# LeonOrou/OPF-Graph-Neural-Solver

Measured on AMD Instinct MI355X. Metric: grids/sec (fwd+bwd) on batched case118, K=4, higher is better.
Workload: dtype f32

## Files before the change

opf-graph-neural-solver_amd/csrc/gns_api.hip:

```cpp
#include <atomic>
#include <cmath>
#include <cstring>
#include <cstdlib>
#include <mutex>
#include <vector>
#include "gns_kernels.h"
#include "gns_gridwg.h"

namespace {
struct GnsTuning {
  int fwd_mapping;
  int gw_pack;
  int fwd_waves;
  int fwd_plane;
  int dw_mfma;
  int train_mapping;
  int bwd_variant;
  int team;
  int bwds_mode;
  int bwds_chunks;
  int bwds_save;
};

bool waves_ok(int& w) { return w > 0 && (w & (w - 1)) == 0 && w * 64 <= GNS_FWD_MAX_THREADS; }
bool chunks_ok(int& c) { return c == 0 || gns_part_index(c) >= 0; }
bool as_flag(int& v) { v = v ? 1 : 0; return true; }
int env_int(const char* e) { return std::atoi(e); }
int env_mapping(const char* e) { return !std::strcmp(e, "lane") ? 1 : (!std::strcmp(e, "lds") ? 2 : 0); }
int env_plane(const char* e) { return e[0] == '0' ? 0 : (e[0] == '1' ? 1 : 2); }
int env_flag(const char* e) { return e[0] == '0' ? 0 : 1; }
struct GnsOption {
  const char* name; int GnsTuning::*member; int lo, hi; bool (*check)(int&); const char* env; int (*parse)(const char*);
  bool accepts(int& v) const { return check ? check(v) : (v >= lo && v <= hi); }
};
const GnsOption g_options[] = {
  {"fwd_mapping",   &GnsTuning::fwd_mapping,   0, 2,            nullptr,   "GNS_FWD_MAPPING",   env_mapping},
  {"train_mapping", &GnsTuning::train_mapping, 0, 2,            nullptr,   "GNS_TRAIN_MAPPING", env_mapping},
  {"bwd_variant",   &GnsTuning::bwd_variant,   1, 4,            nullptr,   "GNS_BWD_VARIANT",   env_int},
  {"gw_pack",       &GnsTuning::gw_pack,       0, 16,           nullptr,   "GNS_GW_PACK",       env_int},
  {"fwd_waves",     &GnsTuning::fwd_waves,     0, 0,            waves_ok,  "GNS_FWD_WAVES",     env_int},
  {"fwd_plane",     &GnsTuning::fwd_plane,     0, 2,            nullptr,   "GNS_FWD_PLANE",     env_plane},
  {"dw_mfma",       &GnsTuning::dw_mfma,       0, 0,            as_flag,   "GNS_DW_MFMA",       env_flag},
  {"team",          &GnsTuning::team,          0, GNS_MAX_TEAM, nullptr,   "GNS_TEAM",          env_int},
  {"bwds_mode",     &GnsTuning::bwds_mode,     0, 2,            nullptr,   "GNS_BWDS_MODE",     env_int},
  {"bwds_chunks",   &GnsTuning::bwds_chunks,   0, 0,            chunks_ok, "GNS_BWDS_CHUNKS",   env_int},
  {"bwds_save",     &GnsTuning::bwds_save,     0, 1,            nullptr,   "GNS_BWDS_SAVE",     env_int},
};
GnsTuning make_tuning() {
  GnsTuning t{0, 0, GNS_FWD_THREADS / 64, 2, 1, 0, 4, 0, 1, 0, 1};
  for (const GnsOption& o : g_options)
    if (const char* e = std::getenv(o.env)) { int v = o.parse(e); if (o.accepts(v)) t.*o.member = v; }
  return t;
}
GnsTuning& tuning() {
  static GnsTuning t = make_tuning();
  return t;
}

struct GnsLast {
  int fwd_kernel, fwd_waves, fwd_plane, team, gw_pack;
  int bwd_kernel, dw_mfma, bwds_mode, bwds_chunks, bwds_R, bwd_gw_pack;
  int bwds_save;
};
GnsLast g_last{-1, -1, -1, -1, -1, -1, -1, -1, -1, -1, -1, -1};
struct GnsLastName { const char* name; int GnsLast::*member; };
const GnsLastName g_last_names[] = {
  {"fwd_kernel", &GnsLast::fwd_kernel}, {"fwd_waves", &GnsLast::fwd_waves}, {"fwd_plane", &GnsLast::fwd_plane}, {"team", &GnsLast::team},
  {"gw_pack", &GnsLast::gw_pack}, {"bwd_kernel", &GnsLast::bwd_kernel}, {"dw_mfma", &GnsLast::dw_mfma}, {"bwds_mode", &GnsLast::bwds_mode},
  {"bwds_chunks", &GnsLast::bwds_chunks}, {"bwds_R", &GnsLast::bwds_R}, {"bwd_gw_pack", &GnsLast::bwd_gw_pack},
  {"bwds_save", &GnsLast::bwds_save},
};
void record_forward(int kernel, int waves, int plane, int team, int pack) {
  g_last.fwd_kernel = kernel; g_last.fwd_waves = waves; g_last.fwd_plane = plane; g_last.team = team; g_last.gw_pack = pack;
}
void record_backward(int kernel, int dw_mfma, int mode, int chunks, int R, int pack, int save = 0) {
  g_last.bwd_kernel = kernel; g_last.dw_mfma = dw_mfma; g_last.bwds_mode = mode; g_last.bwds_chunks = chunks; g_last.bwds_R = R;
  g_last.bwd_gw_pack = pack; g_last.bwds_save = save;
}

constexpr int GNS_MAX_DEVICES = 64;
struct GnsDevice {
  int ncu;
  int gw_ready;
  int split_ready;
  int fwd_ready;
};
const GnsDevice& device() {
  static GnsDevice devs[GNS_MAX_DEVICES];
  static std::atomic<int> done[GNS_MAX_DEVICES];
  static std::mutex mu;
  static const GnsDevice none{0, 0, 0, 0};
  int dev = 0;
  if (hipGetDevice(&dev) != hipSuccess) { (void)hipGetLastError(); return none; }
  if (dev < 0 || dev >= GNS_MAX_DEVICES) return none;
  if (!done[dev].load(std::memory_order_acquire)) {
    std::lock_guard<std::mutex> lock(mu);
    if (!done[dev].load(std::memory_order_relaxed)) {
      GnsDevice d{0, 0, 0, 0};
      int n = 0;
      if (hipDeviceGetAttribute(&n, hipDeviceAttributeMultiprocessorCount, dev) == hipSuccess) d.ncu = n;
// ... 276 lines not shown
                   const void* packed_inputs, int64_t Bt, const float* grad_total, const float* grad_last, const float* grad_v,
                   const float* grad_theta, float* grad_params, hipStream_t st, const IgradOut* ig = nullptr) {
  const int N = cfg->n_bus, E = cfg->n_line, K = cfg->K, d = cfg->latent_dim, h = cfg->hidden_dim;
  int rc;
  GnsBwdsArgs A;
  std::memset(&A, 0, sizeof(A));
  A.topo = topo_dev; A.group_topo = group_topo; A.slot_grid = slot_grid;
  A.pt = (const float*)(fw + L.off_pt); A.pn = (const float*)(fw + L.off_pn);
  A.in = packed_inputs ? (const float*)packed_inputs : (const float*)(fw + L.off_in);
  A.state = (const float*)(fw + L.off_state); A.lam = (const float*)(fw + L.off_lam); A.msg = (const float*)(fw + L.off_msg);
  A.g_total = grad_total; A.g_last = grad_last; A.g_v = grad_v; A.g_theta = grad_theta;
  A.adj = (float*)(bw + S.off_adj); A.slots = (float*)(bw + S.off_slots); A.slab = (float*)(bw + S.off_slab);
  fill_backward_families(A, fam);
  A.Bt = Bt; A.G = S.groups; A.slab_floats = S.slab_floats; A.N = N; A.E = E; A.K = K;
  A.C = S.C; A.part_idx = gns_part_index(S.C); A.R = S.R;
  A.RB = (int)(1 + S.mq); A.RBA = (int)S.adj_rows;
  A.mode = cfg->multiple_phi ? tuning().bwds_mode : 2;
  const size_t lds = gns_bwds_phys_lds(N, &A.use_plane);
  if (ig) {
    A.igrad = ig->buf;
    if (hipMemsetAsync(A.igrad, 0, ig->bytes, st) != hipSuccess) return GNS_ELAUNCH;
  }
  A.save_a1 = saves_first_layer(cfg, ig ? GNS_SAVE_IGRAD : 1, group_topo != nullptr) ? 1 : 0;
  record_backward(4, 1, A.mode, A.C, A.R, -1, A.save_a1);
  prof_mark(1, true, st);
  for (int k = K - 1; k >= 0; --k) {
    A.k = k;
    A.gwk = loss_weight(cfg, k);
    rc = gns_launch_bwds_phys(A, lds, st);
    if (rc != GNS_OK) return rc;
    if (ig) {
      rc = gns_launch_bwds_igrad_phys(A, st);
      if (rc != GNS_OK) return rc;
    }
    rc = gns_launch_bwds_sweep(d, h, cfg->multiple_phi, A, st);
    if (rc != GNS_OK) return rc;
  }
  if (ig && (ig->buses || ig->lines || ig->gens)) {
    rc = gns_launch_bwds_igrad_unpack(A, ig->in_buses, ig->in_lines, ig->in_gens, cfg->n_gen, ig->buses, ig->lines, ig->gens, st);
    if (rc != GNS_OK) return rc;
  }
  prof_mark(1, false, st);
  if (!grad_params) return GNS_OK;
  return gns_launch_reduce(A.slab, (float*)(bw + S.off_part), (float*)(bw + S.off_tmp), params, grad_params, S.nslab, S.slab_floats,
                           fam, K, d, h, st);
}
}
// ... 434 lines not shown
```

opf-graph-neural-solver_amd/csrc/gns_backward_split.hip:

```cpp
#include "gns_device.h"
#include "gns_kernels.h"
#include "gns_dw.h"
#include "gns_phys_device.h"

typedef int gns_i8v __attribute__((ext_vector_type(8)));
#ifndef GNS_BWDS_ONE_LAYOUT
#define GNS_BWDS_ONE_LAYOUT 0
#endif
#ifndef GNS_BWDS_WPE
#define GNS_BWDS_WPE 2
#endif
#ifndef GNS_BWDS_KEEP_SLOPES
#define GNS_BWDS_KEEP_SLOPES 1
#endif
#if GNS_BWDS_KEEP_SLOPES
#define GNS_SLOPES(sl) sl
#define GNS_SLOPE_OF(sl, layer, act, u) sl[layer][u]
#else
#define GNS_SLOPES(sl) nullptr
#define GNS_SLOPE_OF(sl, layer, act, u) dlrelu2(act[u])
#endif
#ifndef GNS_BWDS_FRESH_INPUTS
#define GNS_BWDS_FRESH_INPUTS 1
#endif
#ifndef GNS_BWDS_LINE_AHEAD
#define GNS_BWDS_LINE_AHEAD 1
#endif
#ifndef GNS_BWDS_BUS_AHEAD
#define GNS_BWDS_BUS_AHEAD 1
#endif
#ifndef GNS_BWDS_AH_M
#define GNS_BWDS_AH_M 5
#endif
#ifndef GNS_BWDS_AH_M0
#define GNS_BWDS_AH_M0 5
#endif
#ifndef GNS_BWDS_AH_T0
#define GNS_BWDS_AH_T0 4
#endif
#ifndef GNS_BWDS_LASTK_FOLD
#define GNS_BWDS_LASTK_FOLD 0
#endif
#define GNS_BWDS_PHYS_THREADS (GNS_BWDS_PHYS_WAVES * 64)

__global__ void __launch_bounds__(GNS_BWDS_PHYS_THREADS) gns_bwds_phys_kernel(GnsBwdsArgs A) {
  extern __shared__ __attribute__((aligned(16))) float lds[];
  constexpr int W = GNS_BWDS_PHYS_WAVES;
  const int lane = threadIdx.x & 63;
  const int wave = __builtin_amdgcn_readfirstlane(threadIdx.x >> 6);
  const int N = A.N, E = A.E, K = A.K, k = A.k;
  cip topo = (cip)A.topo;
  const long long g = blockIdx.x;
  long long b = g * GNS_LANES + lane;
  bool live = b < A.Bt;
  if (A.group_topo) {
    const int s = A.slot_grid[g * GNS_LANES + lane];
    b = s;
    live = s >= 0 && s < A.Bt;
    if (!gns_group_topo(A.topo, A.group_topo, g, N, E, topo)) return;
  }
  constexpr int pidx = 4;
// ... 206 lines not shown
  static constexpr bool FOLD4 = WIDE && l < 2 && XT + H + 1 <= 16;
  static constexpr bool FOLDM = GwSubWide::NA >= 16 && WIDE && l == 2 && XT + H + 1 <= 16 && H + (OUT - 16) <= 16;

  static constexpr int NT4 = FOLD4 ? 1 : (FOLDM ? 1 : NA4);
  f32x4 T1[NB1], T2, T4[NT4];
  cfp nb, ptl;

  __device__ __forceinline__ void init(const GnsBwdsArgs& A) {
    const long long koff = A.k;
    nb = (cfp)A.pn + A.n_off[C::NPHI + l] + koff * A.n_sz[C::NPHI + l];
    ptl = (cfp)A.pt + A.t_off[C::NPHI + l] + koff * A.t_sz[C::NPHI + l];
    scalar_cache_warm(ptl, A.t_sz[C::NPHI + l]);
#if !GNS_BWDS_ONE_LAYOUT
    scalar_cache_warm(nb, A.n_sz[C::NPHI + l]);
#endif
    const f32x4 z4 = {0.f, 0.f, 0.f, 0.f};
#pragma unroll
    for (int t = 0; t < NB1; ++t) T1[t] = z4;
#pragma unroll
    for (int t = 0; t < NT4; ++t) T4[t] = z4;
    T2 = z4;
  }

  template <bool ACC_GS, bool STEP0, bool IG = false, bool SV = false>
  __device__ __forceinline__ void bus(const GnsBwdsArgs& A, float* rec, int lane, long long g, int n, float g3s, f2 (&xs)[XL],
                                      f2 (&macc)[D / 2], f4& xsum, f2 (&gS)[H / 2], float* park = nullptr) {
    static_assert(!SV || (MULTI && !GNS_BWDS_ONE_LAYOUT && WIDE && 2 * SOFF >= 16 && (FOLD4 || FOLDM)), "saved activations: the (20, 10) windows");
    f2 (&S)[H / 2] = reinterpret_cast<f2 (&)[H / 2]>(xs[SOFF]);
    f2 a1[H / 2], a2[H / 2], g2[H / 2], g1[H / 2];
    if constexpr (SV) load_pairs<H>(A.msg, ((((long long)A.k * A.G + g) * A.N + n) * C::NPHI + fphi) * C::HQ, lane, a1);
    else load_pairs<H>(A.msg, ((((long long)A.k * A.G + g) * A.N + n) * C::NPHI + fphi) * C::HQ, lane, S);
    WFirst wf;
    f2 sl[2][H / 2];
    using TL [[maybe_unused]] = TLay<LIN, H, OUTP>;
#if GNS_BWDS_ONE_LAYOUT
    (void)wf;
    mlp2_fwd<LIN, H>(ptl, xs, a1, a2, NoBG{}, NoLink{}, GNS_SLOPES(sl));
#else
    using LKm = std::conditional_t<STEP0, NoLink, L2>; using LKs = std::conditional_t<STEP0, std::conditional_t<FOLD4, L0, NoLink>, std::conditional_t<FOLD4, L1, L2>>;
    if constexpr (SV) {
      mlp2_fwd_l2<LIN, H>(ptl, a1, a2, std::conditional_t<STEP0, NoLink, L0>{nullptr, nb, &wf}, GNS_SLOPES(sl));
    } else if constexpr (STEP0) {
      f2 u4[H / 2];
      const f2 (&st)[2] = reinterpret_cast<const f2 (&)[2]>(xs[0]);
      const f2 (&tl)[(LIN - 4 - D + 1) / 2] = reinterpret_cast<const f2 (&)[(LIN - 4 - D + 1) / 2]>(xs[SOFF]);
      phi_head<4, H>(ptl, st, u4);
      phi_tail<LIN, H, 4 + D>(ptl, u4, tl, a1, a2, NoBG{}, NoLink{}, GNS_SLOPES(sl));
    } else {
      mlp2_fwd<LIN, H>(ptl, xs, a1, a2, NoBG{}, L0{nullptr, nb, &wf}, GNS_SLOPES(sl));
    }
#endif
#if GNS_BWDS_ONE_LAYOUT
    if constexpr (l == 2) {
// ... 107 lines not shown

  __device__ __forceinline__ void flush(const GnsBwdsArgs& A, int lane, float* slab) {
    const long long koff = A.k;
    constexpr int ob1 = LIN * H, oW2 = ob1 + H, ob2 = oW2 + H * H, oW4 = ob2 + H, ob4 = oW4 + OUT * H;
    float* lb_ = slab + A.g_off[C::NPHI + l] + koff * A.g_sz[C::NPHI + l];
    static_for<0, NB1>([&](auto t_) { constexpr int t = decltype(t_)::value;
      gws_flush(lane, T1[t], lb_, [&](int c, int il) {
        const bool lastw = WIDE && t == NB1 - 1;
        const int i = 16 * t + il;
        if (c < H) return (lastw && il >= XT) ? -1 : (i < LIN ? c * LIN + i : (i == LIN ? ob1 + c : -1));
        if (FOLD4 && lastw && c == H && il >= XT && il <= XT + H) return il - XT < H ? oW4 + (il - XT) : ob4;
        if (FOLDM && lastw && c >= H && c < H + (OUT - 16) && il >= XT && il <= XT + H) { const int j = 16 + c - H; return il - XT < H ? oW4 + j * H + (il - XT) : ob4 + j; }
        return -1; }, true); });
    gws_flush(lane, T2, lb_, [&](int c, int il) { return c < H ? (il < H ? oW2 + c * H + il : (il == H ? ob2 + c : -1)) : -1; }, true);
    if constexpr (FOLDM)
      gws_flush(lane, T4[0], lb_, [&](int c, int il) { return il < H ? oW4 + c * H + il : (il == H ? ob4 + c : -1); }, true);
    else if constexpr (!FOLD4)
    static_for<0, NA4>([&](auto t_) { constexpr int t = decltype(t_)::value;
      gws_flush(lane, T4[t], lb_, [&](int c, int il) { const int j = 12 * t + c; return (c < 12 && j < OUT) ? (il < H ? oW4 + j * H + il : (il == H ? ob4 + j : -1)) : -1; }, true); });
  }
};

struct BwdsLineRows { f4 a, b; };
__device__ __forceinline__ BwdsLineRows bwds_line_rows(const float* IN, long long row_ein, int p, int lane) {
  return BwdsLineRows{*row_ptr(IN, row_ein + 3LL * p, lane), *row_ptr(IN, row_ein + 3LL * p + 1, lane)};
}

template <int D, int H, bool MULTI, int PF>
struct BwdsPhi : BwdsShape<D, H, MULTI> {
  using B = BwdsShape<D, H, MULTI>;
  using C = typename B::C;
  using SW = typename B::SW;
  using L0 = typename B::L0; using L2 = typename B::L2;
  static constexpr int XL = B::XL, PIN = B::PIN, NDM = B::NDM, NDMF = B::NDMF;
  static constexpr bool WIDE = B::WIDE;

  f32x4 TP1, TP2, TPm[NDMF];
  cfp pnb, ptb;

  __device__ __forceinline__ void init(const GnsBwdsArgs& A) {
    const long long koff = A.k;
    pnb = (cfp)A.pn + A.n_off[PF] + koff * A.n_sz[PF];
    ptb = (cfp)A.pt + A.t_off[PF] + koff * A.t_sz[PF];
    scalar_cache_warm(ptb, A.t_sz[PF]);
#if !GNS_BWDS_ONE_LAYOUT
    scalar_cache_warm(pnb, A.n_sz[PF]);
#endif
    const f32x4 z4 = {0.f, 0.f, 0.f, 0.f};
#pragma unroll
    for (int t = 0; t < NDMF; ++t) TPm[t] = z4;
    TP1 = z4; TP2 = z4;
  }

  template <bool STEP0, bool IG = false, bool LA = false, bool SV = false>
  __device__ __forceinline__ void bus(const GnsBwdsArgs& A, float* rec, int lane, const f2 (&xs)[XL], const f2 (&gS)[H / 2],
                                      f2 (&macc)[D / 2], int p0, int p1, long long row_ein, const BwdsLineRows& first) {
    if (p0 >= p1) return;
    const float* IN = A.in;
    const f2 (&m)[D / 2] = reinterpret_cast<const f2 (&)[D / 2]>(xs[2]);
    WFirst wf;
    (void)wf;
    f2 uh[H / 2], G1[H / 2];
    if constexpr (WIDE)
      static_for<0, (D - 16) / 2>([&](auto j_) { constexpr int j = decltype(j_)::value; gws_putB<SW>(rec, lane, 8 + (PIN - D + 2) / 2 + j, m[8 + j]); });
    if constexpr (STEP0) {
#pragma unroll
      for (int j = 0; j < H / 2; ++j) uh[j] = f2{0.f, 0.f};
    } else {
      phi_head<D, H>(ptb, m, uh);
    }
#pragma unroll
    for (int j = 0; j < H / 2; ++j) G1[j] = f2{0.f, 0.f};
    f4 ca, cb;
    if constexpr (LA) { ca = first.a; cb = first.b; }
    for (int p = p0; p < p1; ++p) {
      f4 na, nb, ea, eb;
      if constexpr (LA) {
        na = *row_ptr(IN, row_ein + 3LL * min(p + 1, p1 - 1), lane); nb = *row_ptr(IN, row_ein + 3LL * min(p + 1, p1 - 1) + 1, lane);
        ea = ca; eb = cb;
      } else {
        ea = *row_ptr(IN, row_ein + 3LL * p, lane); eb = *row_ptr(IN, row_ein + 3LL * p + 1, lane);
      }
      const f2 xt[3] = {f2{ea.x, ea.y}, f2{ea.z, ea.w}, f2{eb.x, 0.f}};
      f2 a1[H / 2], a2[H / 2], g2[H / 2], g1[H / 2];
      f2 sl[2][H / 2];
#if GNS_BWDS_ONE_LAYOUT
      phi_tail<PIN, H, D>(ptb, uh, xt, a1, a2, NoBG{}, NoLink{}, GNS_SLOPES(sl));
#pragma unroll
      for (int u = 0; u < H / 2; ++u) g2[u] = gS[u] * GNS_SLOPE_OF(sl, 1, a2, u);
      bwd_rows_fwd_layout<H, H>(ptb + TLay2<PIN, H>::oW2, g2, g1);
#else
      phi_tail<PIN, H, D>(ptb, uh, xt, a1, a2, NoBG{}, L0{nullptr, pnb, &wf}, GNS_SLOPES(sl));
      if constexpr (SV) {
        f2* const S = const_cast<f2*>(&xs[B::SOFF]);
#pragma unroll
        for (int u = 0; u < H / 2; ++u) S[u] += a2[u];
      }
#pragma unroll
      for (int u = 0; u < H / 2; ++u) g2[u] = gS[u] * GNS_SLOPE_OF(sl, 1, a2, u);
      bwd_rows<H, H>(pnb, g2, g1, NoBG{}, L2{&wf, nullptr, nullptr});
#endif
// ... 53 lines not shown
    gws_flush(lane, TP2, pb_, [&](int c, int il) { return c < H ? (il < H ? pW2 + c * H + il : (il == H ? pb2 + c : -1)) : -1; }, true);
    static_for<0, NDMF>([&](auto t_) { constexpr int t = decltype(t_)::value;
      gws_flush(lane, TPm[t], pb_, [&](int c, int il) { const int i = 16 * t + il; return (c < H && i < D) ? c * PIN + i : -1; }, true); });
  }
};

template <int D, int H, bool MULTI, int FAMS, bool GROUPED, bool IG>
struct BwdsMeasured { static constexpr bool value = MULTI && D == 20 && H == 10 && (FAMS == 3 || FAMS == 4) && !GROUPED && !IG; };
template <int D>
struct BwdsTop { f4 a0, s0; f2 m[D / 2], q0[D / 2], q2[D / 2]; };
template <int D, int H, bool MULTI, int FAMS, bool STEP0, bool GROUPED, bool IG>
struct BwdsAhead {
#if GNS_BWDS_BUS_AHEAD
  static constexpr int value = !BwdsMeasured<D, H, MULTI, FAMS, GROUPED, IG>::value ? 0 : (FAMS == 4 ? (STEP0 ? GNS_BWDS_AH_M0 : GNS_BWDS_AH_M) : (STEP0 ? GNS_BWDS_AH_T0 : 0));
#else
  static constexpr int value = 0;
#endif
};

template <bool SV, int H> struct BwdsPark { static __device__ __forceinline__ float* get() { return nullptr; } };
template <int H> struct BwdsPark<true, H> {
  static __device__ __forceinline__ float* get() { __shared__ __attribute__((aligned(16))) float park[2 * H * GNS_LANES]; return park; }
};
template <int D, int H, bool MULTI, int FAMS, bool STEP0, bool GROUPED, bool IG, bool SV = false>
__global__ void __launch_bounds__(64) __attribute__((amdgpu_waves_per_eu(GNS_BWDS_WPE))) gns_bwds_sweep_kernel(GnsBwdsArgs A) {
  static_assert(!SV || BwdsMeasured<D, H, MULTI, FAMS, GROUPED, IG>::value, "saved activations: the measured shape only");
  using C = GnsDims<D, H, MULTI>;
  static_assert(MULTI || FAMS == 7, "the single phi is reversed after all three L nets");
  constexpr int RB = C::RB, MQ = C::MQ, RBA = 4 + 6 * MQ;
  constexpr bool HAS_T = FAMS & 1, HAS_V = FAMS & 2, HAS_M = FAMS & 4;
  constexpr int SLOT = HAS_M ? 2 : (HAS_T ? 0 : 1);
  constexpr int LIN = C::LF_IN, XL = (LIN + 1) / 2;
  constexpr int RECF = 64 * (D > 16 ? GwSubWide::RS : GwSub::RS);
  __shared__ __attribute__((aligned(16))) float rec[RECF];
  float* const park = BwdsPark<SV, H>::get();
  const int lane = threadIdx.x;
  const long long GB = (A.G + A.R - 1) / A.R;
  const long long bid = blockIdx.x;
  const long long gb = bid % GB;
  const int c = (int)(bid / GB);
  const int N = A.N, E = A.E, K = A.K, k = A.k;
  cip topo = (cip)A.topo;
  cip part = topo + topo[TH_PART] + A.part_idx * (GNS_MAXP + 1), in_ptr = topo + topo[TH_IN_PTR], is_gen = topo + topo[TH_IS_GEN];
  int n0 = part[c], n1 = part[c + 1];
  const long long g0 = gb * A.R, g1 = (g0 + A.R < A.G) ? g0 + A.R : A.G;
  float* slab = A.slab + (gb * A.C + c) * A.slab_floats;
  const bool lastk = k == K - 1;
  constexpr bool LA = BwdsMeasured<D, H, MULTI, FAMS, GROUPED, IG>::value && (GNS_BWDS_LINE_AHEAD == 1 || (GNS_BWDS_LINE_AHEAD == 2 && FAMS == 4));
  constexpr bool ZERO_M = HAS_M || (GNS_BWDS_LASTK_FOLD && MULTI && HAS_T && !GROUPED && !IG);
  if (ZERO_M && lastk) {
    float* z0 = slab + A.g_off[C::NPHI + 2] + (long long)(K - 1) * A.g_sz[C::NPHI + 2];
    for (int i = lane; i < (int)A.g_sz[C::NPHI + 2]; i += 64) z0[i] = 0.f;
    if constexpr (MULTI) {
      float* z1 = slab + A.g_off[2] + (long long)(K - 1) * A.g_sz[2];
      for (int i = lane; i < (int)A.g_sz[2]; i += 64) z1[i] = 0.f;
    }
    if (!HAS_T && !HAS_V) return;
  }
// ... 2 lines not shown
  BwdsL<D, H, MULTI, 1> lv;
  BwdsPhi<D, H, MULTI, MULTI ? 2 : 0> pm;
  BwdsPhi<D, H, MULTI, MULTI ? 1 : 0> pt;
  BwdsPhi<D, H, MULTI, 0> pv;
  if constexpr (HAS_M) { lm.init(A); pm.init(A); }
  if constexpr (HAS_T) { lt.init(A); if constexpr (MULTI) pt.init(A); }
  if constexpr (HAS_V) { lv.init(A); if constexpr (MULTI) pv.init(A); }
  constexpr bool step0 = STEP0;
  const int par = k & 1, parn = par ^ 1;
  const bool m2_live = (A.mode == 2) || k + 1 < K - 1;
  const long long R = gns_in_rows(N, E);

  for (long long g = g0; g < g1; ++g) {
    if constexpr (GROUPED) {
      if (!gns_group_topo(A.topo, A.group_topo, g, N, E, topo)) continue;
      part = topo + topo[TH_PART] + A.part_idx * (GNS_MAXP + 1); in_ptr = topo + topo[TH_IN_PTR]; is_gen = topo + topo[TH_IS_GEN];
      n0 = part[c]; n1 = part[c + 1];
    }
    const long long row_ein = g * R + 3LL * N;
    auto state_row = [&](int slot, int n) { return (((long long)slot * A.G + g) * N + n) * RB; };
    constexpr int AH = BwdsAhead<D, H, MULTI, FAMS, STEP0, GROUPED, IG>::value;
    auto request = [&](int nn, BwdsTop<D>& t) {
      const long long arn = (g * N + nn) * RBA, mrn = arn + 4 + (long long)parn * 3 * MQ;
      if constexpr (AH & 4) { t.a0 = *row_ptr(A.adj, arn, lane); t.s0 = *row_ptr(A.state, state_row(k, nn), lane); }
      if constexpr (AH & 2) load_pairs<D>(A.state, state_row(k, nn) + 1, lane, t.m);
      if constexpr (AH & 1) { load_pairs<D>(A.adj, mrn, lane, t.q0); load_pairs<D>(A.adj, mrn + (m2_live ? 2 : 0) * MQ, lane, t.q2); }
    };
    BwdsTop<D> nx;
    if constexpr (AH != 0) { if (n0 < n1) request(n0, nx); }
    for (int n = n0; n < n1; ++n) {
      const long long ar = (g * N + n) * RBA, rr = state_row(k, n);
      const f4 a0 = [&]() { if constexpr (AH & 4) return nx.a0; else return *row_ptr(A.adj, ar, lane); }();
      const f4 s0 = [&]() { if constexpr (AH & 4) return nx.s0; else return *row_ptr(A.state, rr, lane); }();
      f2 xs[XL];
      f2 (&m)[D / 2] = reinterpret_cast<f2 (&)[D / 2]>(xs[2]);
      if constexpr (AH & 2) {
#pragma unroll
        for (int i = 0; i < D / 2; ++i) m[i] = nx.m[i];
      } else {
        load_pairs<D>(A.state, (step0 ? state_row(0, n0) : rr) + 1, lane, m);
      }
      f2 macc[D / 2];
      if (HAS_M && !lastk) {
        const long long mr = ar + 4 + (long long)parn * 3 * MQ;
        if (A.mode == 2) {
          load_pairs<D>(A.adj, mr + 2 * MQ, lane, macc);
        } else {
          f2 p0v[D / 2];
          if constexpr (AH & 1) {
#pragma unroll
            for (int i = 0; i < D / 2; ++i) { p0v[i] = nx.q0[i]; macc[i] = nx.q2[i]; }
          } else {
            load_pairs<D>(A.adj, mr, lane, p0v);
            load_pairs<D>(A.adj, mr + (m2_live ? 2 : 0) * MQ, lane, macc);
          }
          if (A.mode == 0) {
            f2 p1v[D / 2];
            load_pairs<D>(A.adj, mr + MQ, lane, p1v);
#pragma unroll
            for (int i = 0; i < D / 2; ++i) macc[i] = m2_live ? (macc[i] + p0v[i]) + p1v[i] : p0v[i] + p1v[i];
          } else {
#pragma unroll
            for (int i = 0; i < D / 2; ++i) macc[i] = m2_live ? macc[i] + p0v[i] : p0v[i];
          }
        }
      } else {
#pragma unroll
        for (int i = 0; i < D / 2; ++i) macc[i] = f2{0.f, 0.f};
      }
      auto ahead = [&]() { if constexpr (AH != 0) request(min(n + 1, n1 - 1), nx); };
      f4 xsum = f4{0.f, 0.f, 0.f, 0.f};
      const int p0 = in_ptr[n], p1 = in_ptr[n + 1];
      xs[0] = f2{s0.x, s0.y}; xs[1] = f2{s0.z, s0.w};
      xs[XL - 1] = f2{(float)(p1 - p0), 1.f};
      f2 gS[H / 2];
      const float g3v = is_gen[n] ? 0.f : a0.x;
      auto fresh = [&]() {
#if GNS_BWDS_FRESH_INPUTS
        pin_all(xs);
#endif
      };
      BwdsLineRows lr;
      auto first = [&]() { if constexpr (LA) lr = bwds_line_rows(A.in, row_ein, max(min(p0, E - 1), 0), lane); };
      constexpr int SOFF = 2 + D / 2;
      auto zs = [&]() {
        if constexpr (SV) {
#pragma unroll
          for (int j = 0; j < H / 2; ++j) xs[SOFF + j] = f2{0.f, 0.f};
        }
      };
      if constexpr (MULTI) {
        if constexpr (HAS_M) { if (!lastk) { first(); zs(); fresh(); lm.template bus<false, STEP0, IG, SV>(A, rec, lane, g, n, 0.f, xs, macc, xsum, gS, park); ahead(); fresh(); pm.template bus<STEP0, IG, LA, SV>(A, rec, lane, xs, gS, macc, p0, p1, row_ein, lr); if constexpr (SV) lm.finish(rec, park, lane, xs); } }
        if constexpr (HAS_T) { first(); zs(); fresh(); lt.template bus<false, STEP0, IG, SV>(A, rec, lane, g, n, a0.y, xs, macc, xsum, gS, park); if constexpr (!HAS_M) ahead(); fresh(); pt.template bus<STEP0, IG, LA, SV>(A, rec, lane, xs, gS, macc, p0, p1, row_ein, lr); if constexpr (SV) lt.finish(rec, park, lane, xs); }
        if constexpr (HAS_V) { if (!is_gen[n]) { first(); zs(); fresh(); lv.template bus<false, STEP0, IG, SV>(A, rec, lane, g, n, g3v, xs, macc, xsum, gS, park); fresh(); pv.template bus<STEP0, IG, LA, SV>(A, rec, lane, xs, gS, macc, p0, p1, row_ein, lr); if constexpr (SV) lv.finish(rec, park, lane, xs); } }
      } else {
#pragma unroll
        for (int j = 0; j < H / 2; ++j) gS[j] = f2{0.f, 0.f};
        if (!lastk) { fresh(); lm.template bus<true, STEP0, IG>(A, rec, lane, g, n, 0.f, xs, macc, xsum, gS); }
        first(); fresh(); lt.template bus<true, STEP0, IG>(A, rec, lane, g, n, a0.y, xs, macc, xsum, gS);
        if (!is_gen[n]) { fresh(); lv.template bus<true, STEP0, IG>(A, rec, lane, g, n, g3v, xs, macc, xsum, gS); }
        fresh(); pm.template bus<STEP0, IG, LA>(A, rec, lane, xs, gS, macc, p0, p1, row_ein, lr);
      }
      if constexpr (!step0) {
        *row_ptr(A.adj, ar + 1 + SLOT, lane) = xsum;
        store_pairs<D>(A.adj, ar + 4 + (par * 3 + SLOT) * MQ, lane, macc);
      } else if constexpr (IG) {
        *row_ptr(A.adj, ar + 1 + SLOT, lane) = xsum;
      }
    }
  }
  if constexpr (HAS_M) { if (!lastk) lm.flush(A, lane, slab); if (MULTI ? !lastk : true) pm.flush(A, lane, slab); }
  if constexpr (HAS_T) { lt.flush(A, lane, slab); if constexpr (MULTI) pt.flush(A, lane, slab); }
  if constexpr (HAS_V) { lv.flush(A, lane, slab); if constexpr (MULTI) pv.flush(A, lane, slab); }
}

__global__ void __launch_bounds__(GNS_BWDS_PHYS_THREADS) gns_bwds_igrad_phys_kernel(GnsBwdsArgs A) {
  __shared__ float red[GNS_BWDS_PHYS_WAVES * GNS_LANES];
  constexpr int W = GNS_BWDS_PHYS_WAVES;
  const int lane = threadIdx.x & 63;
  const int wave = __builtin_amdgcn_readfirstlane(threadIdx.x >> 6);
  const int N = A.N, E = A.E, k = A.k;
  cip topo = (cip)A.topo;
  const long long g = blockIdx.x;
  constexpr int pidx = 4;
  const cip in_ptr = topo + topo[TH_IN_PTR], out_ptr = topo + topo[TH_OUT_PTR], q2p = topo + topo[TH_Q2P], is_gen = topo + topo[TH_IS_GEN],
// ... 185 lines not shown

size_t gns_bwds_phys_lds(int N, int* use_plane) {
  const size_t red = (size_t)GNS_BWDS_PHYS_WAVES * GNS_LANES * 4;
  const size_t plane = (size_t)N * GNS_LANES * 4;
  const int level = red + 3 * plane <= (size_t)160 * 1024 ? 2 : (red + 2 * plane <= (size_t)160 * 1024 ? 1 : 0);
  if (use_plane) *use_plane = level;
  return red + (level == 2 ? 3 : (level == 1 ? 2 : 0)) * plane;
}

int gns_launch_bwds_phys(const GnsBwdsArgs& A, size_t lds, hipStream_t st) {
  hipLaunchKernelGGL(gns_bwds_phys_kernel, dim3((unsigned)A.G), dim3(GNS_BWDS_PHYS_THREADS), lds, st, A);
  return hipGetLastError() == hipSuccess ? GNS_OK : GNS_ELAUNCH;
}

int gns_launch_bwds_sweep(int d, int h, int multi, const GnsBwdsArgs& A, hipStream_t st) {
  const long long GB = (A.G + A.R - 1) / A.R;
  const unsigned blocks = (unsigned)(GB * A.C);
  const bool fold_m = GNS_BWDS_LASTK_FOLD && A.k == A.K - 1 && !A.group_topo && !A.igrad;
#define GNS_SWEEP1(DD, HH, MM, FAMS, GR, IG) do { if (A.k == 0) hipLaunchKernelGGL((gns_bwds_sweep_kernel<DD, HH, MM, FAMS, true, GR, IG>), dim3(blocks), dim3(64), 0, st, A); \
                                                 else hipLaunchKernelGGL((gns_bwds_sweep_kernel<DD, HH, MM, FAMS, false, GR, IG>), dim3(blocks), dim3(64), 0, st, A); } while (0)
#define GNS_SWEEP(DD, HH, MM, FAMS) do { if (A.group_topo) GNS_SWEEP1(DD, HH, MM, FAMS, true, false); \
                                         else if (A.igrad) GNS_SWEEP1(DD, HH, MM, FAMS, false, true); \
                                         else GNS_SWEEP1(DD, HH, MM, FAMS, false, false); } while (0)
  if (A.save_a1) {
    if (d != 20 || h != 10 || !multi || A.mode != 1 || A.group_topo || A.igrad) return GNS_EINVAL;
#define GNS_SAVED(FAMS) do { if (A.k == 0) hipLaunchKernelGGL((gns_bwds_sweep_kernel<20, 10, true, FAMS, true, false, false, true>), dim3(blocks), dim3(64), 0, st, A); \
                             else hipLaunchKernelGGL((gns_bwds_sweep_kernel<20, 10, true, FAMS, false, false, false, true>), dim3(blocks), dim3(64), 0, st, A); } while (0)
    if (!fold_m) GNS_SAVED(4);
    GNS_SAVED(3);
#undef GNS_SAVED
    return hipGetLastError() == hipSuccess ? GNS_OK : GNS_ELAUNCH;
  }
#define GNS_CASE(DD, HH)                                                                                                    \
  if (d == DD && h == HH) {                                                                                                 \
    if (!multi) { if (A.mode != 2) return GNS_EINVAL; GNS_SWEEP(DD, HH, false, 7); }                                        \
    else if (A.mode == 2) GNS_SWEEP(DD, HH, true, 7);                                                                       \
    else if (A.mode == 1) { if (!fold_m) GNS_SWEEP(DD, HH, true, 4); GNS_SWEEP(DD, HH, true, 3); }                          \
    else { if (!fold_m) GNS_SWEEP(DD, HH, true, 4); GNS_SWEEP(DD, HH, true, 1); GNS_SWEEP(DD, HH, true, 2); }               \
    return hipGetLastError() == hipSuccess ? GNS_OK : GNS_ELAUNCH;                                                          \
  }
  GNS_FOR_EACH_DIMS(GNS_CASE)
#undef GNS_CASE
#undef GNS_SWEEP
#undef GNS_SWEEP1
  return GNS_EUNSUPPORTED;
}

int gns_bwds_init_device() {
  return hipFuncSetAttribute((const void*)gns_bwds_phys_kernel, hipFuncAttributeMaxDynamicSharedMemorySize, 160 * 1024) == hipSuccess
             ? GNS_OK : GNS_ELAUNCH;
}
```

opf-graph-neural-solver_amd/csrc/gns_device.h:

```cpp
#pragma once
#include <hip/hip_runtime.h>
#include <type_traits>
#include "gns_common.h"

typedef float f2 __attribute__((ext_vector_type(2)));
typedef float f4 __attribute__((ext_vector_type(4)));
typedef float f16v __attribute__((ext_vector_type(16)));
typedef const __attribute__((address_space(4))) float* cfp;
typedef const __attribute__((address_space(4))) int* cip;

__device__ __forceinline__ bool gns_group_topo(const int* set, const int* group_topo, long long g, int N, int E, cip& topo) {
  topo = (cip)set + ((cip)group_topo)[g];
  return topo[TH_MAGIC] == GNS_TOPO_MAGIC && topo[TH_N] == N && topo[TH_E] == E;
}
typedef const __attribute__((address_space(4))) f16v* cf16p;
typedef f16v f16u __attribute__((aligned(4)));
typedef const __attribute__((address_space(4))) f16u* cf16up;

struct GnsTeam {
  unsigned* ctr;
  float* red;
  int size, member;
  unsigned epoch;
  int* failed;
// ... 484 lines not shown
    const f4 t = *row_ptr(base, row + q, lane);
    m[2 * q] = f2{t.x, t.y};
    if constexpr (2 * q + 1 < D / 2) m[2 * q + 1] = f2{t.z, t.w};
  });
}
template <int D>
__device__ __forceinline__ void store_pairs_nt(float* base, long long row, int lane, const f2 (&m)[D / 2]) {
  static_for<0, (D + 3) / 4>([&](auto q_) {
    constexpr int q = decltype(q_)::value;
    f4 t = {m[2 * q].x, m[2 * q].y, 0.f, 0.f};
    if constexpr (2 * q + 1 < D / 2) { t.z = m[2 * q + 1].x; t.w = m[2 * q + 1].y; }
    __builtin_nontemporal_store(t, row_ptr(base, row + q, lane));
  });
}
template <int D>
__device__ __forceinline__ void store_pairs(float* base, long long row, int lane, const f2 (&m)[D / 2]) {
  static_for<0, (D + 3) / 4>([&](auto q_) {
    constexpr int q = decltype(q_)::value;
    f4 t = {m[2 * q].x, m[2 * q].y, 0.f, 0.f};
    if constexpr (2 * q + 1 < D / 2) { t.z = m[2 * q + 1].x; t.w = m[2 * q + 1].y; }
    *row_ptr(base, row + q, lane) = t;
  });
}
```

opf-graph-neural-solver_amd/csrc/gns_kernels.h:

```cpp
#pragma once
#include <hip/hip_runtime.h>
#include "../../include/gns_hip.h"
#include "gns_common.h"

#define GNS_FWD_THREADS 1024
#define GNS_FWD_MAX_THREADS 1024
#define GNS_BWD_THREADS 512
#define GNS_MAX_K 64
#define GNS_FWD_RED_BYTES (2 * GNS_MAXW * GNS_LANES * 2 * 4)
#define GNS_FWD_DYN_LDS_MAX (160 * 1024 - 64)
static inline int gns_fwd_plane_fits(int N, int team) {
  return (size_t)N * GNS_LANES * 8 + (team == 1 ? GNS_FWD_RED_BYTES : 0) <= (size_t)GNS_FWD_DYN_LDS_MAX;
}
static inline int gns_fwd_plane2_fits(int N, int team) {
  return team == 1 && 2 * (size_t)N * GNS_LANES * 8 + GNS_FWD_RED_BYTES <= (size_t)GNS_FWD_DYN_LDS_MAX;
}

#define GNS_FOR_EACH_DIMS(X) X(20, 14) X(20, 10) X(10, 10)
#define GNS_FOR_EACH_DIMS_PERSISTENT(X) X(20, 10) X(10, 10)
#define GNS_FOR_EACH_DIMS_GWB(X) X(20, 10) X(10, 10)

template <int D, int H, bool MULTI>
struct GnsDims {
  static constexpr int NPHI = MULTI ? 3 : 1;
// ... 56 lines not shown
int gns_launch_pack_params(const float* flat, float* pt, float* pn, const GnsFamilies& fam, int K, int D, int H, hipStream_t st);
int gns_launch_pack_inputs(const int* topo, const float* buses, const float* lines, const float* gens, float* out, int N,
                           int E, int Gn, long long Bt, long long groups, hipStream_t st,
                           const int* group_topo = nullptr, const int* slot_grid = nullptr);

struct GnsBwdsArgs {
  const int* topo;
  const float* pt; const float* pn;
  const float* in; const float* state; const float* lam; const float* msg;
  const float* g_total; const float* g_last; const float* g_v; const float* g_theta;
  float* adj; float* slots; float* slab;
  long long t_off[6], t_sz[6], n_off[6], n_sz[6], g_off[6], g_sz[6];
  long long Bt, G, slab_floats;
  float gwk;
  int N, E, K, k;
  int C, part_idx, R;
  int RB, RBA;
  int use_plane;
  int mode;
  const int* group_topo;
  const int* slot_grid;
  float* igrad;
  int save_a1;
};
int gns_bwds_supported(int d, int h, int multi);
size_t gns_bwds_phys_lds(int N, int* use_plane);
int gns_launch_bwds_phys(const GnsBwdsArgs& A, size_t lds, hipStream_t st);
int gns_launch_bwds_sweep(int d, int h, int multi, const GnsBwdsArgs& A, hipStream_t st);
int gns_launch_bwds_igrad_phys(const GnsBwdsArgs& A, hipStream_t st);
int gns_launch_bwds_igrad_unpack(const GnsBwdsArgs& A, const float* buses, const float* lines, const float* gens, int Gn,
                                 float* grad_buses, float* grad_lines, float* grad_gens, hipStream_t st);
int gns_bwds_init_device();
```

Baseline: 6.254 million.

## Stage saved first-layer activations into LDS via async global-to-LDS loads in sweeps

Adds a staged variant of the saved-activation backward sweep kernel. It prefetches the next node's first-layer activations directly into LDS with global_load_lds_dwordx4, so the load overlaps the current node's compute. It also narrows the adjacency and line-row loads to the components actually used, and moves the register pinning point later. The variant is on by default when save_a1 is set. It adds inline asm with manual m0 handling and vmcnt waits, and the s_waitcnt vmcnt(0) may also stall on unrelated outstanding loads.

```diff
diff --git a/opf-graph-neural-solver_amd/csrc/gns_api.hip b/opf-graph-neural-solver_amd/csrc/gns_api.hip
--- a/opf-graph-neural-solver_amd/csrc/gns_api.hip
+++ b/opf-graph-neural-solver_amd/csrc/gns_api.hip
@@ -20,6 +20,7 @@
   int bwds_mode;
   int bwds_chunks;
   int bwds_save;
+  int bwds_stage;
 };
 
 bool waves_ok(int& w) { return w > 0 && (w & (w - 1)) == 0 && w * 64 <= GNS_FWD_MAX_THREADS; }
@@ -45,9 +46,10 @@
   {"bwds_mode",     &GnsTuning::bwds_mode,     0, 2,            nullptr,   "GNS_BWDS_MODE",     env_int},
   {"bwds_chunks",   &GnsTuning::bwds_chunks,   0, 0,            chunks_ok, "GNS_BWDS_CHUNKS",   env_int},
   {"bwds_save",     &GnsTuning::bwds_save,     0, 1,            nullptr,   "GNS_BWDS_SAVE",     env_int},
+  {"bwds_stage",    &GnsTuning::bwds_stage,    0, 1,            nullptr,   "GNS_BWDS_STAGE",    env_int},
 };
 GnsTuning make_tuning() {
-  GnsTuning t{0, 0, GNS_FWD_THREADS / 64, 2, 1, 0, 4, 0, 1, 0, 1};
+  GnsTuning t{0, 0, GNS_FWD_THREADS / 64, 2, 1, 0, 4, 0, 1, 0, 1, 1};
   for (const GnsOption& o : g_options)
     if (const char* e = std::getenv(o.env)) { int v = o.parse(e); if (o.accepts(v)) t.*o.member = v; }
   return t;
@@ -61,21 +63,22 @@
   int fwd_kernel, fwd_waves, fwd_plane, team, gw_pack;
   int bwd_kernel, dw_mfma, bwds_mode, bwds_chunks, bwds_R, bwd_gw_pack;
   int bwds_save;
-};
-GnsLast g_last{-1, -1, -1, -1, -1, -1, -1, -1, -1, -1, -1, -1};
+  int bwds_stage;
+};
+GnsLast g_last{-1, -1, -1, -1, -1, -1, -1, -1, -1, -1, -1, -1, -1};
 struct GnsLastName { const char* name; int GnsLast::*member; };
 const GnsLastName g_last_names[] = {
   {"fwd_kernel", &GnsLast::fwd_kernel}, {"fwd_waves", &GnsLast::fwd_waves}, {"fwd_plane", &GnsLast::fwd_plane}, {"team", &GnsLast::team},
   {"gw_pack", &GnsLast::gw_pack}, {"bwd_kernel", &GnsLast::bwd_kernel}, {"dw_mfma", &GnsLast::dw_mfma}, {"bwds_mode", &GnsLast::bwds_mode},
   {"bwds_chunks", &GnsLast::bwds_chunks}, {"bwds_R", &GnsLast::bwds_R}, {"bwd_gw_pack", &GnsLast::bwd_gw_pack},
-  {"bwds_save", &GnsLast::bwds_save},
+  {"bwds_save", &GnsLast::bwds_save}, {"bwds_stage", &GnsLast::bwds_stage},
 };
 void record_forward(int kernel, int waves, int plane, int team, int pack) {
   g_last.fwd_kernel = kernel; g_last.fwd_waves = waves; g_last.fwd_plane = plane; g_last.team = team; g_last.gw_pack = pack;
 }
-void record_backward(int kernel, int dw_mfma, int mode, int chunks, int R, int pack, int save = 0) {
+void record_backward(int kernel, int dw_mfma, int mode, int chunks, int R, int pack, int save = 0, int stage = 0) {
   g_last.bwd_kernel = kernel; g_last.dw_mfma = dw_mfma; g_last.bwds_mode = mode; g_last.bwds_chunks = chunks; g_last.bwds_R = R;
-  g_last.bwd_gw_pack = pack; g_last.bwds_save = save;
+  g_last.bwd_gw_pack = pack; g_last.bwds_save = save; g_last.bwds_stage = stage;
 }
 
 constexpr int GNS_MAX_DEVICES = 64;
@@ -398,7 +401,8 @@
     if (hipMemsetAsync(A.igrad, 0, ig->bytes, st) != hipSuccess) return GNS_ELAUNCH;
   }
   A.save_a1 = saves_first_layer(cfg, ig ? GNS_SAVE_IGRAD : 1, group_topo != nullptr) ? 1 : 0;
-  record_backward(4, 1, A.mode, A.C, A.R, -1, A.save_a1);
+  A.stage = (A.save_a1 && tuning().bwds_stage == 1) ? 1 : 0;
+  record_backward(4, 1, A.mode, A.C, A.R, -1, A.save_a1, A.stage);
   prof_mark(1, true, st);
   for (int k = K - 1; k >= 0; --k) {
     A.k = k;
diff --git a/opf-graph-neural-solver_amd/csrc/gns_backward_split.hip b/opf-graph-neural-solver_amd/csrc/gns_backward_split.hip
--- a/opf-graph-neural-solver_amd/csrc/gns_backward_split.hip
+++ b/opf-graph-neural-solver_amd/csrc/gns_backward_split.hip
@@ -37,6 +37,15 @@
 #endif
 #ifndef GNS_BWDS_AH_T0
 #define GNS_BWDS_AH_T0 4
+#endif
+#ifndef GNS_BWDS_STAGE_A1
+#define GNS_BWDS_STAGE_A1 1
+#endif
+#ifndef GNS_BWDS_STAGE_PIN
+#define GNS_BWDS_STAGE_PIN 1
+#endif
+#ifndef GNS_BWDS_STAGE_NARROW
+#define GNS_BWDS_STAGE_NARROW 1
 #endif
 #ifndef GNS_BWDS_LASTK_FOLD
 #define GNS_BWDS_LASTK_FOLD 0
@@ -289,13 +298,17 @@
     T2 = z4;
   }
 
-  template <bool ACC_GS, bool STEP0, bool IG = false, bool SV = false>
+  template <bool ACC_GS, bool STEP0, bool IG = false, bool SV = false, bool STG = false>
   __device__ __forceinline__ void bus(const GnsBwdsArgs& A, float* rec, int lane, long long g, int n, float g3s, f2 (&xs)[XL],
-                                      f2 (&macc)[D / 2], f4& xsum, f2 (&gS)[H / 2], float* park = nullptr) {
+                                      f2 (&macc)[D / 2], f4& xsum, f2 (&gS)[H / 2], float* park = nullptr, const f2* a1s = nullptr) {
+    static_assert(!STG || SV, "staged a1: saved activations only");
     static_assert(!SV || (MULTI && !GNS_BWDS_ONE_LAYOUT && WIDE && 2 * SOFF >= 16 && (FOLD4 || FOLDM)), "saved activations: the (20, 10) windows");
     f2 (&S)[H / 2] = reinterpret_cast<f2 (&)[H / 2]>(xs[SOFF]);
     f2 a1[H / 2], a2[H / 2], g2[H / 2], g1[H / 2];
-    if constexpr (SV) load_pairs<H>(A.msg, ((((long long)A.k * A.G + g) * A.N + n) * C::NPHI + fphi) * C::HQ, lane, a1);
+    if constexpr (STG) {
+#pragma unroll
+      for (int u = 0; u < H / 2; ++u) a1[u] = a1s[u];
+    } else if constexpr (SV) load_pairs<H>(A.msg, ((((long long)A.k * A.G + g) * A.N + n) * C::NPHI + fphi) * C::HQ, lane, a1);
     else load_pairs<H>(A.msg, ((((long long)A.k * A.G + g) * A.N + n) * C::NPHI + fphi) * C::HQ, lane, S);
     WFirst wf;
     f2 sl[2][H / 2];
@@ -449,8 +462,10 @@
 };
 
 struct BwdsLineRows { f4 a, b; };
+template <bool NARROW = false>
 __device__ __forceinline__ BwdsLineRows bwds_line_rows(const float* IN, long long row_ein, int p, int lane) {
-  return BwdsLineRows{*row_ptr(IN, row_ein + 3LL * p, lane), *row_ptr(IN, row_ein + 3LL * p + 1, lane)};
+  if constexpr (NARROW) return BwdsLineRows{*row_ptr(IN, row_ein + 3LL * p, lane), f4{*reinterpret_cast<const float*>(row_ptr(IN, row_ein + 3LL * p + 1, lane)), 0.f, 0.f, 0.f}};
+  else return BwdsLineRows{*row_ptr(IN, row_ein + 3LL * p, lane), *row_ptr(IN, row_ein + 3LL * p + 1, lane)};
 }
 
 template <int D, int H, bool MULTI, int PF>
@@ -479,7 +494,7 @@
     TP1 = z4; TP2 = z4;
   }
 
-  template <bool STEP0, bool IG = false, bool LA = false, bool SV = false>
+  template <bool STEP0, bool IG = false, bool LA = false, bool SV = false, bool NARROW = false>
   __device__ __forceinline__ void bus(const GnsBwdsArgs& A, float* rec, int lane, const f2 (&xs)[XL], const f2 (&gS)[H / 2],
                                       f2 (&macc)[D / 2], int p0, int p1, long long row_ein, const BwdsLineRows& first) {
     if (p0 >= p1) return;
@@ -503,7 +518,9 @@
     for (int p = p0; p < p1; ++p) {
       f4 na, nb, ea, eb;
       if constexpr (LA) {
-        na = *row_ptr(IN, row_ein + 3LL * min(p + 1, p1 - 1), lane); nb = *row_ptr(IN, row_ein + 3LL * min(p + 1, p1 - 1) + 1, lane);
+        na = *row_ptr(IN, row_ein + 3LL * min(p + 1, p1 - 1), lane);
+        if constexpr (NARROW) nb = f4{*reinterpret_cast<const float*>(row_ptr(IN, row_ein + 3LL * min(p + 1, p1 - 1) + 1, lane)), 0.f, 0.f, 0.f};
+        else nb = *row_ptr(IN, row_ein + 3LL * min(p + 1, p1 - 1) + 1, lane);
         ea = ca; eb = cb;
       } else {
         ea = *row_ptr(IN, row_ein + 3LL * p, lane); eb = *row_ptr(IN, row_ein + 3LL * p + 1, lane);
@@ -603,9 +620,15 @@
 template <int H> struct BwdsPark<true, H> {
   static __device__ __forceinline__ float* get() { __shared__ __attribute__((aligned(16))) float park[2 * H * GNS_LANES]; return park; }
 };
-template <int D, int H, bool MULTI, int FAMS, bool STEP0, bool GROUPED, bool IG, bool SV = false>
+template <bool ST> struct BwdsStage { static __device__ __forceinline__ float* get() { return nullptr; } };
+template <> struct BwdsStage<true> {
+  static __device__ __forceinline__ float* get() { __shared__ __attribute__((aligned(16))) float stage[2 * 4 * GNS_LANES]; return stage; }
+};
+template <int D, int H, bool MULTI, int FAMS, bool STEP0, bool GROUPED, bool IG, bool SV = false, bool ST = false>
 __global__ void __launch_bounds__(64) __attribute__((amdgpu_waves_per_eu(GNS_BWDS_WPE))) gns_bwds_sweep_kernel(GnsBwdsArgs A) {
   static_assert(!SV || BwdsMeasured<D, H, MULTI, FAMS, GROUPED, IG>::value, "saved activations: the measured shape only");
+  static_assert(!ST || (SV && H == 10), "staged sweeps: saved activations, a1 = two rows and one pair");
+  constexpr bool STG = ST && GNS_BWDS_STAGE_A1, LATE_PIN = ST && GNS_BWDS_STAGE_PIN, NARROW = ST && GNS_BWDS_STAGE_NARROW;
   using C = GnsDims<D, H, MULTI>;
   static_assert(MULTI || FAMS == 7, "the single phi is reversed after all three L nets");
   constexpr int RB = C::RB, MQ = C::MQ, RBA = 4 + 6 * MQ;
@@ -615,6 +638,7 @@
   constexpr int RECF = 64 * (D > 16 ? GwSubWide::RS : GwSub::RS);
   __shared__ __attribute__((aligned(16))) float rec[RECF];
   float* const park = BwdsPark<SV, H>::get();
+  float* const stage = BwdsStage<STG>::get();
   const int lane = threadIdx.x;
   const long long GB = (A.G + A.R - 1) / A.R;
   const long long bid = blockIdx.x;
@@ -663,15 +687,40 @@
     constexpr int AH = BwdsAhead<D, H, MULTI, FAMS, STEP0, GROUPED, IG>::value;
     auto request = [&](int nn, BwdsTop<D>& t) {
       const long long arn = (g * N + nn) * RBA, mrn = arn + 4 + (long long)parn * 3 * MQ;
-      if constexpr (AH & 4) { t.a0 = *row_ptr(A.adj, arn, lane); t.s0 = *row_ptr(A.state, state_row(k, nn), lane); }
+      if constexpr (AH & 4) {
+        if constexpr (NARROW) { const f2 a = *reinterpret_cast<const f2*>(row_ptr(A.adj, arn, lane)); t.a0 = f4{a.x, a.y, 0.f, 0.f}; }
+        else t.a0 = *row_ptr(A.adj, arn, lane);
+        t.s0 = *row_ptr(A.state, state_row(k, nn), lane);
+      }
       if constexpr (AH & 2) load_pairs<D>(A.state, state_row(k, nn) + 1, lane, t.m);
       if constexpr (AH & 1) { load_pairs<D>(A.adj, mrn, lane, t.q0); load_pairs<D>(A.adj, mrn + (m2_live ? 2 : 0) * MQ, lane, t.q2); }
     };
     BwdsTop<D> nx;
     if constexpr (AH != 0) { if (n0 < n1) request(n0, nx); }
+    constexpr int F0 = HAS_M ? 2 : 1, FV = 0;
+    [[maybe_unused]] f2 a1n[H / 2];
+    [[maybe_unused]] f2 stg_tail;
+    [[maybe_unused]] auto stage_req = [&](int nn, int fphi) {
+      if constexpr (STG) {
+        const long long row = ((((long long)k * A.G + g) * N + nn) * C::NPHI + fphi) * C::HQ;
+        stg_tail = *reinterpret_cast<const f2*>(row_ptr(A.msg, row + 2, lane));
+        stage_request<2>(A.msg, row, lane, stage);
+      }
+    };
+    [[maybe_unused]] auto stage_get = [&]() {
+      if constexpr (STG) {
+        stage_read<2>(stage, lane, reinterpret_cast<f2 (&)[4]>(a1n[0]));
+        a1n[4] = stg_tail;
+      }
+    };
+    if constexpr (STG) { if (n0 < n1) { stage_req(n0, F0); stage_get(); } }
     for (int n = n0; n < n1; ++n) {
       const long long ar = (g * N + n) * RBA, rr = state_row(k, n);
-      const f4 a0 = [&]() { if constexpr (AH & 4) return nx.a0; else return *row_ptr(A.adj, ar, lane); }();
+      const f4 a0 = [&]() {
+        if constexpr (AH & 4) return nx.a0;
+        else if constexpr (NARROW) { const f2 a = *reinterpret_cast<const f2*>(row_ptr(A.adj, ar, lane)); return f4{a.x, a.y, 0.f, 0.f}; }
+        else return *row_ptr(A.adj, ar, lane);
+      }();
       const f4 s0 = [&]() { if constexpr (AH & 4) return nx.s0; else return *row_ptr(A.state, rr, lane); }();
       f2 xs[XL];
       f2 (&m)[D / 2] = reinterpret_cast<f2 (&)[D / 2]>(xs[2]);
@@ -680,6 +729,10 @@
         for (int i = 0; i < D / 2; ++i) m[i] = nx.m[i];
       } else {
         load_pairs<D>(A.state, (step0 ? state_row(0, n0) : rr) + 1, lane, m);
+      }
+      if constexpr (STG) {
+        const bool own_v = HAS_V && !is_gen[n];
+        stage_req(own_v ? n : min(n + 1, n1 - 1), own_v ? FV : F0);
       }
       f2 macc[D / 2];
       if (HAS_M && !lastk) {
@@ -722,7 +775,7 @@
 #endif
       };
       BwdsLineRows lr;
-      auto first = [&]() { if constexpr (LA) lr = bwds_line_rows(A.in, row_ein, max(min(p0, E - 1), 0), lane); };
+      auto first = [&]() { if constexpr (LA) lr = bwds_line_rows<NARROW>(A.in, row_ein, max(min(p0, E - 1), 0), lane); };
       constexpr int SOFF = 2 + D / 2;
       auto zs = [&]() {
         if constexpr (SV) {
@@ -731,9 +784,9 @@
         }
       };
       if constexpr (MULTI) {
-        if constexpr (HAS_M) { if (!lastk) { first(); zs(); fresh(); lm.template bus<false, STEP0, IG, SV>(A, rec, lane, g, n, 0.f, xs, macc, xsum, gS, park); ahead(); fresh(); pm.template bus<STEP0, IG, LA, SV>(A, rec, lane, xs, gS, macc, p0, p1, row_ein, lr); if constexpr (SV) lm.finish(rec, park, lane, xs); } }
-        if constexpr (HAS_T) { first(); zs(); fresh(); lt.template bus<false, STEP0, IG, SV>(A, rec, lane, g, n, a0.y, xs, macc, xsum, gS, park); if constexpr (!HAS_M) ahead(); fresh(); pt.template bus<STEP0, IG, LA, SV>(A, rec, lane, xs, gS, macc, p0, p1, row_ein, lr); if constexpr (SV) lt.finish(rec, park, lane, xs); }
-        if constexpr (HAS_V) { if (!is_gen[n]) { first(); zs(); fresh(); lv.template bus<false, STEP0, IG, SV>(A, rec, lane, g, n, g3v, xs, macc, xsum, gS, park); fresh(); pv.template bus<STEP0, IG, LA, SV>(A, rec, lane, xs, gS, macc, p0, p1, row_ein, lr); if constexpr (SV) lv.finish(rec, park, lane, xs); } }
+        if constexpr (HAS_M) { if (!lastk) { first(); zs(); if constexpr (!LATE_PIN) fresh(); lm.template bus<false, STEP0, IG, SV, STG>(A, rec, lane, g, n, 0.f, xs, macc, xsum, gS, park, a1n); ahead(); fresh(); pm.template bus<STEP0, IG, LA, SV, NARROW>(A, rec, lane, xs, gS, macc, p0, p1, row_ein, lr); if constexpr (SV) lm.finish(rec, park, lane, xs); } }
+        if constexpr (HAS_T) { first(); zs(); if constexpr (!LATE_PIN || HAS_M) fresh(); lt.template bus<false, STEP0, IG, SV, STG>(A, rec, lane, g, n, a0.y, xs, macc, xsum, gS, park, a1n); if constexpr (!HAS_M) ahead(); fresh(); pt.template bus<STEP0, IG, LA, SV, NARROW>(A, rec, lane, xs, gS, macc, p0, p1, row_ein, lr); if constexpr (SV) lt.finish(rec, park, lane, xs); }
+        if constexpr (HAS_V) { if (!is_gen[n]) { if constexpr (STG) { stage_get(); stage_req(min(n + 1, n1 - 1), F0); } first(); zs(); fresh(); lv.template bus<false, STEP0, IG, SV, STG>(A, rec, lane, g, n, g3v, xs, macc, xsum, gS, park, a1n); fresh(); pv.template bus<STEP0, IG, LA, SV, NARROW>(A, rec, lane, xs, gS, macc, p0, p1, row_ein, lr); if constexpr (SV) lv.finish(rec, park, lane, xs); } }
       } else {
 #pragma unroll
         for (int j = 0; j < H / 2; ++j) gS[j] = f2{0.f, 0.f};
@@ -742,6 +795,7 @@
         if (!is_gen[n]) { fresh(); lv.template bus<true, STEP0, IG>(A, rec, lane, g, n, g3v, xs, macc, xsum, gS); }
         fresh(); pm.template bus<STEP0, IG, LA>(A, rec, lane, xs, gS, macc, p0, p1, row_ein, lr);
       }
+      if constexpr (STG) stage_get();
       if constexpr (!step0) {
         *row_ptr(A.adj, ar + 1 + SLOT, lane) = xsum;
         store_pairs<D>(A.adj, ar + 4 + (par * 3 + SLOT) * MQ, lane, macc);
@@ -973,13 +1027,16 @@
 #define GNS_SWEEP(DD, HH, MM, FAMS) do { if (A.group_topo) GNS_SWEEP1(DD, HH, MM, FAMS, true, false); \
                                          else if (A.igrad) GNS_SWEEP1(DD, HH, MM, FAMS, false, true); \
                                          else GNS_SWEEP1(DD, HH, MM, FAMS, false, false); } while (0)
+  if (A.stage && !A.save_a1) return GNS_EINVAL;
   if (A.save_a1) {
     if (d != 20 || h != 10 || !multi || A.mode != 1 || A.group_topo || A.igrad) return GNS_EINVAL;
-#define GNS_SAVED(FAMS) do { if (A.k == 0) hipLaunchKernelGGL((gns_bwds_sweep_kernel<20, 10, true, FAMS, true, false, false, true>), dim3(blocks), dim3(64), 0, st, A); \
-                             else hipLaunchKernelGGL((gns_bwds_sweep_kernel<20, 10, true, FAMS, false, false, false, true>), dim3(blocks), dim3(64), 0, st, A); } while (0)
+#define GNS_SAVED1(FAMS, ST) do { if (A.k == 0) hipLaunchKernelGGL((gns_bwds_sweep_kernel<20, 10, true, FAMS, true, false, false, true, ST>), dim3(blocks), dim3(64), 0, st, A); \
+                                  else hipLaunchKernelGGL((gns_bwds_sweep_kernel<20, 10, true, FAMS, false, false, false, true, ST>), dim3(blocks), dim3(64), 0, st, A); } while (0)
+#define GNS_SAVED(FAMS) do { if (A.stage) GNS_SAVED1(FAMS, true); else GNS_SAVED1(FAMS, false); } while (0)
     if (!fold_m) GNS_SAVED(4);
     GNS_SAVED(3);
 #undef GNS_SAVED
+#undef GNS_SAVED1
     return hipGetLastError() == hipSuccess ? GNS_OK : GNS_ELAUNCH;
   }
 #define GNS_CASE(DD, HH)                                                                                                    \
diff --git a/opf-graph-neural-solver_amd/csrc/gns_device.h b/opf-graph-neural-solver_amd/csrc/gns_device.h
--- a/opf-graph-neural-solver_amd/csrc/gns_device.h
+++ b/opf-graph-neural-solver_amd/csrc/gns_device.h
@@ -530,3 +530,32 @@
     *row_ptr(base, row + q, lane) = t;
   });
 }
+
+template <int ROWS>
+__device__ __forceinline__ void stage_request(const float* base, long long row, int lane, float* slot) {
+  static_assert(ROWS == 2, "the two-row slot of the sweeps");
+  const f4* src = row_ptr(base, row, lane);
+  const unsigned dst = (unsigned)(size_t)(__attribute__((address_space(3))) float*)slot;
+  unsigned keep;
+  asm volatile(
+      "s_waitcnt lgkmcnt(0)\n\t"
+      "s_mov_b32 %0, m0\n\t"
+      "s_mov_b32 m0, %2\n\t"
+      "s_nop 0\n\t"
+      "global_load_lds_dwordx4 %1, off\n\t"
+      "global_load_lds_dwordx4 %1, off offset:1024\n\t"
+      "s_mov_b32 m0, %0"
+      : "=&s"(keep)
+      : "v"(src), "s"(dst)
+      : "memory");
+}
+template <int ROWS>
+__device__ __forceinline__ void stage_read(const float* slot, int lane, f2 (&m)[2 * ROWS]) {
+  asm volatile("s_waitcnt vmcnt(0)" ::: "memory");
+  static_for<0, ROWS>([&](auto q_) {
+    constexpr int q = decltype(q_)::value;
+    const f4 t = reinterpret_cast<const f4*>(slot)[q * GNS_LANES + lane];
+    m[2 * q] = f2{t.x, t.y};
+    m[2 * q + 1] = f2{t.z, t.w};
+  });
+}
diff --git a/opf-graph-neural-solver_amd/csrc/gns_kernels.h b/opf-graph-neural-solver_amd/csrc/gns_kernels.h
--- a/opf-graph-neural-solver_amd/csrc/gns_kernels.h
+++ b/opf-graph-neural-solver_amd/csrc/gns_kernels.h
@@ -102,6 +102,7 @@
   const int* slot_grid;
   float* igrad;
   int save_a1;
+  int stage;
 };
 int gns_bwds_supported(int d, int h, int multi);
 size_t gns_bwds_phys_lds(int N, int* use_plane);
```

Result: no change. 6.263 million (median of 2 runs) (+0.2%).
